# araffin/srl-zoo

Measured on AMD Instinct MI355X. Metric: images/sec (224x224x3) AE+VAE train step, higher is better.
Workload: dtype f32; 1 GPU; synthetic 224x224x3 obs, --losses autoencoder, custom_cnn, state-dim 200, bs=256 per GPU (512 frames fwd+bwd per step per GPU), Adam lr 0.005, normalised fp32 observations resident in HBM; global_batch=256, parallelism=dp1, rccl_ranks=1, devices=1

## Files before the change

include/srlz.h:

```cpp
#ifndef SRLZ_H
#define SRLZ_H

#include <stddef.h>
#include <stdint.h>

#ifdef __cplusplus
extern "C" {
#endif

typedef void* srlz_stream_t;

enum srlz_status {
  SRLZ_OK = 0,
  SRLZ_ERR_BAD_DESC = -1,
  SRLZ_ERR_WORKSPACE = -2,
  SRLZ_ERR_HIP = -3,
  SRLZ_ERR_NULL = -4
};

#define SRLZ_ABI_VERSION 104
int srlz_version(void);
const char* srlz_last_error(void);
int srlz_device_cus(void);

typedef struct {
  int n;
  int hi, wi;
  int ho, wo;
  int ksize;
  int stride;
  int pad;
  int transposed;
  int groups;
} srlz_conv64_desc;

size_t srlz_conv64_packed_floats(void);
int srlz_conv64_pack_weights(const float* w_ref, float* wpack_fwd, float* wpack_bwd,
                             const srlz_conv64_desc* d, srlz_stream_t stream);
int srlz_conv64_fwd_tiles(const srlz_conv64_desc* d);
int srlz_conv64_fwd(const float* x, const float* wpack_fwd, const float* bias, float* y, float* stats_partial,
                    const float* x_bnp, const srlz_conv64_desc* d, srlz_stream_t stream);
typedef struct {
  const float* y;
  const float* bnp;
  const float* sums;
  long long count;
  int training;
  float* dy_out;
} srlz_bn_bwd_operand;
int srlz_conv64_bwd_data(const float* dy, const float* wpack_bwd, float* dx, const srlz_bn_bwd_operand* dy_bn,
                         const srlz_conv64_desc* d, srlz_stream_t stream);
struct srlz_pool_desc_s;
int srlz_conv64_bwd_data_tiles(const srlz_conv64_desc* d);
// ... 309 lines not shown
```

srl-zoo_amd/csrc/common.h:

```cpp
#pragma once
#include <hip/hip_runtime.h>
#include <stdint.h>
#include <stddef.h>
#include "../../include/srlz.h"

typedef float f32x4 __attribute__((ext_vector_type(4)));
typedef float f32x16 __attribute__((ext_vector_type(16)));

void srlz_set_error(const char* fmt, ...);
int srlz_hip_fail(hipError_t e, const char* what);

#define SRLZ_HIP(expr)                                   \
  do {                                                   \
    hipError_t _e = (expr);                              \
    if (_e != hipSuccess) return srlz_hip_fail(_e, #expr); \
  } while (0)

#define SRLZ_MAX_LDS(fn, bytes)                                                                                         \
  do {                                                                                                                  \
    static int srlz_lds_set_ = -1;                                                                                      \
    if ((int)(bytes) > srlz_lds_set_) {                                                                                 \
      SRLZ_HIP(hipFuncSetAttribute((const void*)(fn), hipFuncAttributeMaxDynamicSharedMemorySize, (int)(bytes)));      \
      srlz_lds_set_ = (int)(bytes);                                                                                     \
    }                                                                                                                   \
// ... 117 lines not shown
  __syncthreads();
  if (threadIdx.x < 128) {
    double s = 0.0;
#pragma unroll
    for (int r = 0; r < 16; ++r) s += sm[r][threadIdx.x];
    row[threadIdx.x] = (T)s;
  }
}

template <class F4, class F1>
__device__ __forceinline__ void for_each_quad(long long n, F4 quad, F1 one) {
  const long long n4 = n >> 2, stride = (long long)gridDim.x * blockDim.x, first = (long long)blockIdx.x * blockDim.x + threadIdx.x;
  for (long long i = first; i < n4; i += stride) quad(i);
  for (long long i = n4 * 4 + first; i < n; i += stride) one(i);
}
```

srl-zoo_amd/csrc/conv64.hip:

```cpp
#include "conv64_tile.h"
#include <stdlib.h>

static int floordiv(int a, int b) { return (a >= 0) ? a / b : -((-a + b - 1) / b); }

int conv64::build_program(Prog* P, int gather, int stride, int pad, int N, int Hs, int Ws, int Hd, int Wd, int G) {
  if (stride != 1 && stride != 2) return -1;
  if (G < 1 || N % G != 0) return -1;
  N /= G;
  P->N = N; P->Hs = Hs; P->Ws = Ws; P->Hd = Hd; P->Wd = Wd;
  P->G = G;
  P->src_gstride = (long long)N * Hs * Ws * 64;
  P->dst_gstride = (long long)N * Hd * Wd * 64;
  int kcls[3], kd[3];
  if (gather) {
    P->ss = stride; P->ds = 1;
    for (int k = 0; k < 3; ++k) {
      int t = k - pad;
      int c = ((t % stride) + stride) % stride;
      kcls[k] = c; kd[k] = (t - c) / stride;
    }
  } else {
    P->ss = 1; P->ds = stride;
    for (int k = 0; k < 3; ++k) {
      int py = (((k - pad) % stride) + stride) % stride;
// ... 361 lines not shown
}

template <int PSUM>
__global__ __launch_bounds__(256, 2) void conv64_dgrad_poolsum_kernel(const float* __restrict__ src,
                                                                     const float* __restrict__ wpack,
                                                                     float* __restrict__ dst,
                                                                     float* __restrict__ bn_bwd_partial, const ConvProg P,
                                                                     int ntiles, const PoolSum ps) {
  conv64_fwd_body<4, false, PSUM>(src, wpack, nullptr, dst, bn_bwd_partial, P, ntiles, SRLZ_NO_FUSE, ps);
}

__global__ void conv64_pack_kernel(const float* __restrict__ w_ref, float* __restrict__ pf, float* __restrict__ pb,
                                   int transposed) {
  const int id = blockIdx.x * blockDim.x + threadIdx.x;
  if (id >= NTAPS * 4096) return;
  const int tap = id >> 12, n = (id >> 6) & 63, k = id & 63;
  const int o = (tap * 64 + n) * 64 + ((((k >> 2) ^ (n & 15)) << 2) | (k & 3));
  const int fwd_idx = transposed ? ((k * 64 + n) * 9 + tap) : ((n * 64 + k) * 9 + tap);
  const int bwd_idx = transposed ? ((n * 64 + k) * 9 + tap) : ((k * 64 + n) * 9 + tap);
  if (pf) pf[o] = w_ref[fwd_idx];
  if (pb) pb[o] = w_ref[bwd_idx];
}

static int check_desc(const srlz_conv64_desc* d) {
  SRLZ_REQUIRE(d != nullptr, SRLZ_ERR_NULL, "conv64: null descriptor");
  SRLZ_REQUIRE(d->ksize == 3 && (d->stride == 1 || d->stride == 2) && d->n > 0, SRLZ_ERR_BAD_DESC,
               "conv64: only 3x3 stride 1/2 supported (k=%d s=%d)", d->ksize, d->stride);
  SRLZ_REQUIRE(d->groups >= 0 && (d->groups <= 1 || d->n % d->groups == 0), SRLZ_ERR_BAD_DESC,
               "conv64: n = %d is not a multiple of groups = %d", d->n, d->groups);
  int eho, ewo;
  if (!d->transposed) {
    eho = (d->hi + 2 * d->pad - 3) / d->stride + 1;
    ewo = (d->wi + 2 * d->pad - 3) / d->stride + 1;
  } else {
    eho = (d->hi - 1) * d->stride - 2 * d->pad + 3;
    ewo = (d->wi - 1) * d->stride - 2 * d->pad + 3;
// ... 55 lines not shown
  SRLZ_REQUIRE(rc == 0, SRLZ_ERR_BAD_DESC, "conv64: cannot build a grid program for this descriptor");
  return 0;
}

extern "C" size_t srlz_conv64_packed_floats(void) { return (size_t)NTAPS * 4096; }

extern "C" int srlz_conv64_pack_weights(const float* w_ref, float* wpack_fwd, float* wpack_bwd,
                                        const srlz_conv64_desc* d, srlz_stream_t stream) {
  if (int rc = check_desc(d)) return rc;
  SRLZ_REQUIRE(w_ref, SRLZ_ERR_NULL, "conv64_pack: null weights");
  SRLZ_LAUNCH(conv64_pack_kernel, dim3((NTAPS * 4096 + 255) / 256), dim3(256), 0, as_stream(stream), w_ref, wpack_fwd, wpack_bwd,
              d->transposed);
  return 0;
}

extern "C" int srlz_conv64_fwd_tiles(const srlz_conv64_desc* d) {
  ConvProg P;
  if (conv64::with_program(d, 0, &P)) return -1;
  return P.G * P.tpg;
}

extern "C" int srlz_conv64_fwd(const float* x, const float* wpack_fwd, const float* bias, float* y,
                               float* stats_partial, const float* x_bnp, const srlz_conv64_desc* d,
                               srlz_stream_t stream) {
  ConvProg P;
  if (int rc = conv64::with_program(d, 0, &P)) return rc;
  SRLZ_REQUIRE(x && wpack_fwd && y, SRLZ_ERR_NULL, "conv64_fwd: null pointer");
  return launch_fwd(x, wpack_fwd, bias, y, stats_partial, P, as_stream(stream), OpFuse{x_bnp, nullptr, nullptr, 0.f, 0, nullptr});
}

// ... 44 lines not shown
```

srl-zoo_amd/csrc/linear.hip:

```cpp
#include "common.h"

namespace {

constexpr int BR = 32;
constexpr int LD = 68;

__global__ __launch_bounds__(256) void gemm_strided_kernel(const float* __restrict__ A, long long sai, long long sar,
                                                          const float* __restrict__ B, long long sbr, long long sbj,
                                                          const float* __restrict__ bias, float* __restrict__ C, int I,
                                                          int J, int R, int relu, int rchunk, const float* __restrict__ res,
                                                          long long ldr) {
  __shared__ float As[2][BR][LD];
  __shared__ float Bs[2][BR][LD];
  const int tid = threadIdx.x, lane = tid & 63, wave = tid >> 6;
  const int h = lane >> 5, l31 = lane & 31;
  const int wi = wave & 1, wj = wave >> 1;
  const int i0 = blockIdx.y * 64, j0 = blockIdx.x * 64;
  f32x16 acc;
#pragma unroll
  for (int r = 0; r < 16; ++r) acc[r] = 0.f;

  const int rbeg = blockIdx.z * rchunk;
  const int rend = (rbeg + rchunk < R) ? rbeg + rchunk : R;
  C += (size_t)blockIdx.z * I * J;
// ... 52 lines not shown
#pragma unroll
  for (int r = 0; r < 16; ++r) {
    const int i = i0 + wi * 32 + (r & 3) + 8 * (r >> 2) + 4 * h;
    if (i < I && j < J) {
      float v = acc[r] + bj;
      if (relu) v = v > 0.f ? v : 0.f;
      if (res) v = __fadd_rn(v, res[(long long)i * ldr + j]);
      C[(long long)i * J + j] = v;
    }
  }
}

constexpr int TR = 64;
__device__ __forceinline__ int tile_key(int row) { return ((row & 3) << 2) | ((row >> 2) & 3); }

template <bool AI, bool BI>
__global__ __launch_bounds__(256, 2) void gemm_vec_kernel(const float* __restrict__ A, long long lda, const float* __restrict__ B,
                                                         long long ldb, const float* __restrict__ bias, float* __restrict__ C,
                                                         int I, int J, int R, int relu, int rchunk, const float* __restrict__ res,
                                                         long long ldr) {
  __shared__ __attribute__((aligned(16))) float As[2][64 * TR];
  __shared__ __attribute__((aligned(16))) float Bs[2][64 * TR];
  const int tid = threadIdx.x, lane = tid & 63, wave = tid >> 6;
  const int h = lane >> 5, l31 = lane & 31;
  const int wi = wave & 1, wj = wave >> 1;
  const int i0 = blockIdx.y * 64, j0 = blockIdx.x * 64;
  f32x16 acc;
#pragma unroll
  for (int r = 0; r < 16; ++r) acc[r] = 0.f;
  const int rbeg = blockIdx.z * rchunk;
  const int rend = (rbeg + rchunk < R) ? rbeg + rchunk : R;
  C += (size_t)blockIdx.z * I * J;

  f32x4 va[4], vb[4];
  unsigned ina = 0, inb = 0;
// ... 6 lines not shown
      long long off;
      bool ok;
      if (!along_row) {
        const int row = e >> 4, r = 4 * (e & 15);
        ok = row0 + row < nrow && r0 + r < rend;
        off = (long long)(row0 + row) * ld + (r0 + r);
      } else {
        const int r = 4 * (e >> 6) + (e & 3), row = 4 * ((e >> 2) & 15);
        ok = row0 + row < nrow && r0 + r < rend;
        off = (long long)(r0 + r) * ld + (row0 + row);
      }
      v[u] = *(const f32x4*)(P + (ok ? off : 0LL));
      in |= (ok ? 1u : 0u) << u;
    }
  };
  auto stash_one = [&](float* __restrict__ T, bool along_row, const f32x4 (&v)[4], unsigned in) {
#pragma unroll
    for (int u = 0; u < 4; ++u) {
      const int e = tid + 256 * u;
      const f32x4 x = ((in >> u) & 1u) ? v[u] : f32x4{0.f, 0.f, 0.f, 0.f};
      if (!along_row) {
        const int row = e >> 4, slot = e & 15;
        *(f32x4*)(T + row * TR + ((slot ^ tile_key(row)) << 2)) = x;
      } else {
        const int r = 4 * (e >> 6) + (e & 3), row = 4 * ((e >> 2) & 15);
#pragma unroll
        for (int c = 0; c < 4; ++c) T[(row + c) * TR + ((((r >> 2) ^ tile_key(row + c)) << 2) | (r & 3))] = x[c];
      }
    }
  };
  fetch_one(A, lda, AI, i0, I, rbeg, va, ina);
  fetch_one(B, ldb, BI, j0, J, rbeg, vb, inb);
  stash_one(As[0], AI, va, ina);
  stash_one(Bs[0], BI, vb, inb);
  __syncthreads();
  int buf = 0;
  const int arow = wi * 32 + l31, brow = wj * 32 + l31;
  const int akey = tile_key(arow), bkey = tile_key(brow);
  for (int r0 = rbeg; r0 < rend; r0 += TR) {
    const int rn = (r0 + TR < rend) ? r0 + TR : rend;
    fetch_one(A, lda, AI, i0, I, rn, va, ina);
    fetch_one(B, ldb, BI, j0, J, rn, vb, inb);
    __builtin_amdgcn_sched_barrier(0);
    const float* Ab = As[buf] + arow * TR;
    const float* Bb = Bs[buf] + brow * TR;
#pragma unroll
    for (int c = 0; c < TR / 8; ++c) {
      const f32x4 a = *(const f32x4*)(Ab + (((2 * c + h) ^ akey) << 2));
      const f32x4 b = *(const f32x4*)(Bb + (((2 * c + h) ^ bkey) << 2));
#pragma unroll
      for (int m = 0; m < 4; ++m) acc = __builtin_amdgcn_mfma_f32_32x32x2f32(a[m], b[m], acc, 0, 0, 0);
    }
    stash_one(As[buf ^ 1], AI, va, ina);
    stash_one(Bs[buf ^ 1], BI, vb, inb);
    __syncthreads();
    buf ^= 1;
  }
  const int j = j0 + wj * 32 + l31;
  float bj = bias ? bias[j < J ? j : 0] : 0.f;
  asm volatile("" : "+v"(bj));
#pragma unroll
  for (int r = 0; r < 16; ++r) {
    const int i = i0 + wi * 32 + (r & 3) + 8 * (r >> 2) + 4 * h;
    if (i < I && j < J) {
      float v = acc[r] + bj;
      if (relu) v = v > 0.f ? v : 0.f;
      if (res) v = __fadd_rn(v, res[(long long)i * ldr + j]);
      C[(long long)i * J + j] = v;
    }
  }
}

__global__ void splitk_combine_kernel(const float* __restrict__ partial, int nsplit, const float* __restrict__ bias,
                                      float* __restrict__ C, int I, int J, int relu, const float* __restrict__ res, long long ldr) {
  const int e = blockIdx.x * blockDim.x + threadIdx.x;
  if (e >= I * J) return;
  float s = 0.f;
  for (int z = 0; z < nsplit; ++z) s += partial[(size_t)z * I * J + e];
  if (bias) s += bias[e % J];
  if (relu) s = s > 0.f ? s : 0.f;
  if (res) s = __fadd_rn(s, res[(long long)(e / J) * ldr + e % J]);
  C[e] = s;
}

// ... 30 lines not shown
  if (s > R / 128) s = R / 128;
  if (s > 16) s = 16;
  while (s > 1 && (size_t)s * I * J * sizeof(float) > ws_bytes) --s;
  return s < 1 ? 1 : s;
}

static bool vec_ok(const float* P, long long s_row, long long s_r, int nrow, int R, bool* along_row, long long* ld) {
  if (((uintptr_t)P & 15) != 0 || R % 4 != 0) return false;
  if (s_r == 1 && s_row % 4 == 0) { *along_row = false; *ld = s_row; return true; }
  if (s_row == 1 && s_r % 4 == 0 && nrow % 4 == 0) { *along_row = true; *ld = s_r; return true; }
  return false;
}

static int launch(const float* A, long long sai, long long sar, const float* B, long long sbr, long long sbj,
                  const float* bias, float* C, int I, int J, int R, int relu, void* ws, size_t ws_bytes, hipStream_t st,
                  const float* res = nullptr, long long ldr = 0) {
  SRLZ_REQUIRE(I > 0 && J > 0 && R > 0, SRLZ_ERR_BAD_DESC, "linear: empty GEMM %dx%dx%d", I, J, R);
  bool ai = false, bi = false;
  long long lda = 0, ldb = 0;
  const bool vec = vec_ok(A, sai, sar, I, R, &ai, &lda) && vec_ok(B, sbj, sbr, J, R, &bi, &ldb);
  const int step = vec ? TR : BR;
  int splits = ws ? choose_splits(I, J, R, ws_bytes, vec) : 1;
  int rchunk = R, nz = 1;
  if (splits > 1) {
    rchunk = (R + splits - 1) / splits;
    rchunk = (rchunk + step - 1) / step * step;
    nz = (R + rchunk - 1) / rchunk;
  }
  const dim3 grid((J + 63) / 64, (I + 63) / 64, nz);
  const float* kbias = nz > 1 ? nullptr : bias;
  float* kC = nz > 1 ? (float*)ws : C;
  const int krelu = nz > 1 ? 0 : relu;
  const float* kres = nz > 1 ? nullptr : res;
  if (vec) {
#define SRLZ_VEC_LAUNCH(AIV, BIV) \
    SRLZ_LAUNCH((gemm_vec_kernel<AIV, BIV>), grid, dim3(256), 0, st, A, lda, B, ldb, kbias, kC, I, J, R, krelu, rchunk, kres, ldr)
    if (ai && bi) SRLZ_VEC_LAUNCH(true, true);
    else if (ai) SRLZ_VEC_LAUNCH(true, false);
    else if (bi) SRLZ_VEC_LAUNCH(false, true);
    else SRLZ_VEC_LAUNCH(false, false);
#undef SRLZ_VEC_LAUNCH
  } else {
    SRLZ_LAUNCH(gemm_strided_kernel, grid, dim3(256), 0, st, A, sai, sar, B, sbr, sbj, kbias, kC, I, J, R, krelu, rchunk, kres, ldr);
  }
  if (nz > 1) {
    SRLZ_LAUNCH(splitk_combine_kernel, dim3((I * J + 255) / 256), dim3(256), 0, st, (const float*)ws, nz, bias, C, I, J, relu, res, ldr);
  }
  return 0;
}

}

// ... 20 lines not shown
                                        void* ws, size_t ws_bytes, srlz_stream_t stream) {
  SRLZ_REQUIRE(dy && w && dx && res, SRLZ_ERR_NULL, "linear_bwd_data_res: null pointer");
  SRLZ_REQUIRE(Kout >= 1 && Kout <= K, SRLZ_ERR_BAD_DESC, "linear_bwd_data_res: %d of %d input columns", Kout, K);
  return launch(dy, N, 1, w, K, 1, nullptr, dx, M, Kout, N, 0, ws, ws_bytes, as_stream(stream), res, Kout);
}

extern "C" int srlz_linear_bwd_data(const float* dy, const float* w, float* dx, int M, int N, int K, void* ws,
                                    size_t ws_bytes, srlz_stream_t stream) {
  SRLZ_REQUIRE(dy && w && dx, SRLZ_ERR_NULL, "linear_bwd_data: null pointer");
  return launch(dy, N, 1, w, K, 1, nullptr, dx, M, K, N, 0, ws, ws_bytes, as_stream(stream));
}

extern "C" int srlz_linear_bwd_weight(const float* dy, const float* x, float* dw, float* db, int M, int N, int K,
                                      void* ws, size_t ws_bytes, srlz_stream_t stream) {
  SRLZ_REQUIRE(dy && x && dw, SRLZ_ERR_NULL, "linear_bwd_weight: null pointer");
  if (int rc = launch(dy, 1, N, x, K, 1, nullptr, dw, N, K, M, 0, ws, ws_bytes, as_stream(stream))) return rc;
  if (db) {
    SRLZ_LAUNCH(colsum_kernel, dim3((N + 63) / 64), dim3(256), 0, as_stream(stream), dy, db, M, N);
  }
  return 0;
}

extern "C" int srlz_relu_bwd_inplace(const float* y, float* dy, long long n, srlz_stream_t stream) {
  SRLZ_REQUIRE(y && dy, SRLZ_ERR_NULL, "relu_bwd: null pointer");
  long long blocks = (n + 255) / 256;
  if (blocks > 4096) blocks = 4096;
  if (blocks < 1) blocks = 1;
  SRLZ_LAUNCH(relu_bwd_kernel, dim3((int)blocks), dim3(256), 0, as_stream(stream), y, dy, n);
  return 0;
}
```

srl-zoo_amd/csrc/wino.hip:

```cpp
#include "common.h"

namespace {

typedef float f32x2 __attribute__((ext_vector_type(2)));
typedef unsigned u32x2 __attribute__((ext_vector_type(2)));

constexpr int WN_THREADS = 256;
constexpr int WN_TP = 32;
constexpr int WN_CHUNK = 16 * 4 * 64 * 4;
constexpr int WN_VCHUNK = 16 * 4 * WN_TP * 4;
constexpr int WN_VCOMP = 4 * WN_TP * 4;
constexpr unsigned WN_DROP = 0x80000000u;

struct WinoProg {
  int N, G;
  int H, W;
  int PA, PB;
  int ppi, ppg, tpg;
  unsigned mPPI, mPB;
  int sPPI, sPB;
  long long gstride;
};

__global__ void conv64_wino_pack_kernel(const float* __restrict__ w_ref, float* __restrict__ uf, float* __restrict__ ub) {
  const int id = blockIdx.x * blockDim.x + threadIdx.x;
  if (id >= 64 * 64) return;
  const int e = id & 3, m = (id >> 2) & 63, gq = (id >> 8) & 3, p = id >> 10;
  const int k = 16 * p + 4 * gq + e;
#pragma unroll
  for (int dir = 0; dir < 2; ++dir) {
    float* out = dir ? ub : uf;
    if (!out) continue;
    float gk[3][3];
#pragma unroll
    for (int ky = 0; ky < 3; ++ky)
#pragma unroll
      for (int kx = 0; kx < 3; ++kx)
        gk[ky][kx] = dir ? w_ref[((k * 64 + m) * 3 + (2 - ky)) * 3 + (2 - kx)] : w_ref[((m * 64 + k) * 3 + ky) * 3 + kx];
    float t[3][4];
#pragma unroll
    for (int ky = 0; ky < 3; ++ky) {
      t[ky][0] = gk[ky][0];
      t[ky][1] = 0.5f * (gk[ky][0] + gk[ky][1] + gk[ky][2]);
      t[ky][2] = 0.5f * (gk[ky][0] - gk[ky][1] + gk[ky][2]);
      t[ky][3] = gk[ky][2];
    }
#pragma unroll
    for (int nu = 0; nu < 4; ++nu) {
      const float u0 = t[0][nu];
      const float u1 = 0.5f * (t[0][nu] + t[1][nu] + t[2][nu]);
      const float u2 = 0.5f * (t[0][nu] - t[1][nu] + t[2][nu]);
      const float u3 = t[2][nu];
      const float u[4] = {u0, u1, u2, u3};
#pragma unroll
      for (int xi = 0; xi < 4; ++xi) out[(size_t)p * WN_CHUNK + (((xi * 4 + nu) * 4 + gq) * 64 + m) * 4 + e] = u[xi];
    }
  }
}

struct WinoRaw { f32x2 d[16]; f32x2 sc, sh; };

struct WinoPatch {
  unsigned vtop, vmid, vbot;
  bool lef, rig;
};

__device__ __forceinline__ void wn_patch(WinoPatch& wp, const WinoProg& P, int tile_in_group, int t_pt, int t_cp, int* ptab_slot) {
  const int pl = tile_in_group * WN_TP + t_pt;
  const bool ok = pl < P.ppg;
  const int n = fastdiv(pl, P.mPPI, P.sPPI);
  const int rem = pl - n * P.ppi;
  const int a = fastdiv(rem, P.mPB, P.sPB);
// ... 698 lines not shown
```

srl-zoo_amd/models/models.py:

```python
from __future__ import print_function, division, absolute_import

import torch as th
import torch.nn as nn

try:
    from preprocessing.preprocess import getNChannels
except ImportError:
    from ..preprocessing.preprocess import getNChannels

from srlz import hotpath, ops


def conv3x3(in_planes, out_planes, stride=1):
    return nn.Conv2d(in_planes, out_planes, kernel_size=3, stride=stride, padding=1, bias=False)


def _encoder_stack():
    spec = [(nn.Conv2d(getNChannels(), 64, kernel_size=7, stride=2, padding=3, bias=False), 1),
            (conv3x3(64, 64, stride=1), 0),
            (conv3x3(64, 64, stride=2), 0)]
    layers = []
    for conv, pool_pad in spec:
        layers += [conv, nn.BatchNorm2d(64), nn.ReLU(inplace=True), nn.MaxPool2d(kernel_size=3, stride=2, padding=pool_pad)]
    return nn.Sequential(*layers)
# ... 26 lines not shown
    if isinstance(out, tuple):
        halves = [ops.pair_split(t) for t in out]
        return tuple(h[0] for h in halves), tuple(h[1] for h in halves)
    return ops.pair_split(out)


class BaseModelAutoEncoder(BaseModelSRL):

    def __init__(self):
        super(BaseModelAutoEncoder, self).__init__()
        self.encoder_conv = _encoder_stack()
        self.decoder_conv = _decoder_stack()

    def _encodeConv(self, x, stat_sink=None):
        hotpath.require_gpu(x, "encoder")
        e = hotpath.encoder_forward(self.encoder_conv, x, self.training, stat_sink)
        return e.view(e.size(0), -1)

    def _decodeConv(self, z):
        return hotpath.decoder_forward(self.decoder_conv, z.view(z.size(0), 64, 6, 6), self.training)

    def getStates(self, observations):
        return self.encode(observations)

    def encode(self, x):
        raise NotImplementedError

    def decode(self, x):
        raise NotImplementedError

    def forward(self, x):
# ... 85 lines not shown
```

srl-zoo_amd/srlz/_cabi.py:

```python
import ctypes
import os
from ctypes import c_int, c_longlong, c_float, c_double, c_void_p, c_size_t, c_char_p, POINTER, Structure

_HERE = os.path.dirname(os.path.abspath(__file__))
LIB_PATH = os.path.join(_HERE, "libsrlz_hip.so")


ABI_VERSION = 104


class SrlzError(RuntimeError):
    pass


class Conv64Desc(Structure):
    _fields_ = [("n", c_int), ("hi", c_int), ("wi", c_int), ("ho", c_int), ("wo", c_int), ("ksize", c_int),
                ("stride", c_int), ("pad", c_int), ("transposed", c_int), ("groups", c_int)]


class SkinnyDesc(Structure):
    _fields_ = [("n", c_int), ("c", c_int), ("himg", c_int), ("wimg", c_int), ("hf", c_int), ("wf", c_int),
                ("kind", c_int), ("groups", c_int)]


class PoolDesc(Structure):
    _fields_ = [("n", c_int), ("h", c_int), ("w", c_int), ("hp", c_int), ("wp", c_int), ("pool_pad", c_int),
                ("out_nchw", c_int), ("groups", c_int)]


class ConvNDesc(Structure):
    _fields_ = [("n", c_int), ("hi", c_int), ("wi", c_int), ("ho", c_int), ("wo", c_int), ("cin", c_int), ("cout", c_int),
                ("ksize", c_int), ("stride", c_int), ("pad", c_int), ("groups", c_int)]

    def __init__(self, n, hi, wi, ho, wo, cin, cout, ksize, stride, pad, groups=1):
        super(ConvNDesc, self).__init__(n, hi, wi, ho, wo, cin, cout, ksize, stride, pad, groups)


class BnReplayItem(Structure):
    _fields_ = [("batch_stat", c_void_p), ("running_mean", c_void_p), ("running_var", c_void_p), ("num_batches_tracked", c_void_p)]


class BnBwdOperand(Structure):
    _fields_ = [("y", c_void_p), ("bnp", c_void_p), ("sums", c_void_p), ("count", c_longlong), ("training", c_int),
                ("dy_out", c_void_p)]


P = c_void_p
_BO = POINTER(BnBwdOperand)
_C64 = POINTER(Conv64Desc)
_SK = POINTER(SkinnyDesc)
_PD = POINTER(PoolDesc)
_CN = POINTER(ConvNDesc)

_PROTOS = {
    "srlz_version": (c_int, []),
    "srlz_last_error": (c_char_p, []),
    "srlz_device_cus": (c_int, []),
    "srlz_conv64_packed_floats": (c_size_t, []),
    "srlz_conv64_pack_weights": (c_int, [P, P, P, _C64, P]),
    "srlz_conv64_fwd_tiles": (c_int, [_C64]),
    "srlz_conv64_fwd": (c_int, [P, P, P, P, P, P, _C64, P]),
    "srlz_conv64_bwd_data": (c_int, [P, P, P, _BO, _C64, P]),
    "srlz_conv64_bwd_weight_workspace": (c_size_t, [_C64]),
    "srlz_conv64_bwd_fused_supported": (c_int, [_C64]),
    "srlz_conv64_gather_pipe_supported": (c_int, [_C64, c_int]),
    "srlz_conv64_bwd_fused_workspace": (c_size_t, [_C64]),
    "srlz_conv64_bwd_fused": (c_int, [P, P, P, _BO, P, P, P, P, P, P, c_size_t, _C64, P]),
    "srlz_conv64_bwd_fused_bn_rows": (c_int, [_C64]),
    "srlz_conv64_wino_supported": (c_int, [_C64]),
    "srlz_conv64_wino_packed_floats": (c_size_t, []),
    "srlz_conv64_wino_pack_weights": (c_int, [P, P, P, P]),
    "srlz_conv64_wino_tiles": (c_int, [_C64]),
    "srlz_conv64_wino_fwd": (c_int, [P, P, P, P, P, P, _C64, P]),
    "srlz_conv64_wino_bwd_data": (c_int, [P, P, P, _C64, P]),
# ... 204 lines not shown
```

srl-zoo_amd/srlz/hotpath.py:

```python
import os
import torch

from . import ops

TAPS = None


OBSERVE = None


def _observe(prefix, idx, t):
    if OBSERVE is not None:
        OBSERVE["%s.%d" % (prefix, idx)] = (t.detach(), tuple(t.grad_fn.saved_tensors) if t.grad_fn is not None else ())
    return t


def _tap(prefix, idx, t):
    if TAPS is not None and t.requires_grad:
        t.retain_grad()
        TAPS["%s.%d" % (prefix, idx)] = t
    return t


_FUSE_ENC_IN = True
# ... 8 lines not shown
_RECON = None


class recon_loss_into(object):
    def __init__(self, target, mean):
        self.target, self.mean, self.loss = target, bool(mean), None

    def __enter__(self):
        global _RECON
        self.prev, _RECON = _RECON, (self if _FUSE_RECON else None)
        return self

    def __exit__(self, *exc):
        global _RECON
        _RECON = self.prev
        return False


def _bn_args(bn):
    bn.running_mean._srlz_tick = bn.num_batches_tracked
    return bn.weight, bn.bias, bn.running_mean, bn.running_var


def encoder_forward(seq, x, training, stat_sink=None, name="encoder_conv"):
    conv1, bn1, conv2, bn2, conv3, bn3 = seq[0], seq[1], seq[4], seq[5], seq[8], seq[9]
    if not _FUSE_ENC_IN:
        x = ops.frames_as_float(x)
    link1 = ops.PoolLink() if TAPS is None else None
    link2 = ops.PoolLink() if TAPS is None else None
    if _FUSE_ENC_IN and not x.requires_grad:
        p, y = ops.EncInFn.apply(x, conv1.weight, *_bn_args(bn1), training, 1, stat_sink, link1)
        _tap(name, 0, y)
        _tap(name, 3, p)
        _observe(name, 3, p)
    else:
        y, st = ops.Conv1Fn.apply(x, conv1.weight, training)
        _tap(name, 0, y)
        p = _tap(name, 3, ops.BNReLUPoolFn.apply(y, st, *_bn_args(bn1), training, 1, False, stat_sink, link1))
        _observe(name, 3, p)
    y, st = ops.Conv64Fn.apply(p, conv2.weight, None, 1, 1, False, training, link1)
    _tap(name, 4, y)
    p = _observe(name, 7, _tap(name, 7, ops.BNReLUPoolFn.apply(y, st, *_bn_args(bn2), training, 0, False, stat_sink, link2)))
    y, st = ops.Conv64Fn.apply(p, conv3.weight, None, 2, 1, False, training, link2)
    _tap(name, 8, y)
    return _observe(name, 11, _tap(name, 11, ops.BNReLUPoolFn.apply(y, st, *_bn_args(bn3), training, 0, True, stat_sink)))


def replay_encoder_bn(seq, stats, group=0):
    bns = (seq[1], seq[5], seq[9])
    items = [(st[128 * group:128 * (group + 1)], bn.running_mean, bn.running_var, bn.num_batches_tracked) for bn, st in zip(bns, stats)]
    ops._ordered_bn_update([bn.running_mean for bn in bns], lambda: ops.bn_replay_many(items))


def decoder_forward(seq, z, training):
    a = ops.ToNHWCFn.apply(z)
    y, st = ops.Conv64Fn.apply(a, seq[0].weight, seq[0].bias, 2, 0, True, training)
    _tap("decoder_conv", 0, y)
    defer = _DEFER_BN_BWD and TAPS is None
    in_link = None
    for bi, ci in ((1, 3), (4, 6), (7, 9)):
        bn, conv = seq[bi], seq[ci]
        if TAPS is not None:
            _record_activation(bi + 1, y, st, bn, training)
        out_link = ops.BwdLink() if defer else None
        y, st = ops.DecBlockFn.apply(y, st, *_bn_args(bn), training, conv.weight, conv.bias, training, in_link, out_link)
        in_link = out_link
        _tap("decoder_conv", ci, y)
        _observe("decoder_conv", ci, y)
    bn, last = seq[10], seq[12]
    if TAPS is not None:
        _record_activation(11, y, st, bn, training)
# ... 165 lines not shown
```

srl-zoo_amd/srlz/ops.py:

```python
import weakref

import torch
from torch.autograd import Function

from . import _cabi as C
from ._cabi import ptr, stream, Conv64Desc, SkinnyDesc, PoolDesc, ConvNDesc

BN_EPS = 1e-5
BN_MOMENTUM = 0.1

_GROUPS = 1


class batch_groups(object):
    def __init__(self, groups):
        self.groups = int(groups)

    def __enter__(self):
        global _GROUPS
        self.prev, _GROUPS = _GROUPS, self.groups
        return self

    def __exit__(self, *exc):
        global _GROUPS
# ... 202 lines not shown

class PoolLink:

    def __init__(self):
        self.record = None
        self.partials = None

    def take_partials(self):
        p, self.partials, self.record = self.partials, None, None
        return p


_POOL_LINK = True


class Conv64Fn(Function):
    @staticmethod
    def forward(ctx, x, w, bias, stride, pad, transposed, want_stats, in_link=None):
        x, w = _check(x, "conv64 input"), _check(w, "conv64 weight")
        n, hi, wi, ch = x.shape
        assert ch == 64 and tuple(w.shape) == (64, 64, 3, 3)
        d = conv64_desc(n, hi, wi, stride, pad, transposed, cur_groups(want_stats))
        y = torch.empty((n, d.ho, d.wo, 64), dtype=torch.float32, device=x.device)
        ctx.wino = bool(C.conv64_wino_supported(d))
        if ctx.wino:
            packs = torch.empty((2, C.conv64_wino_packed_floats()), dtype=torch.float32, device=x.device)
            C.conv64_wino_pack_weights(ptr(w), ptr(packs[0]), ptr(packs[1]), stream())
            stats = torch.empty((C.conv64_wino_tiles(d), 128), dtype=torch.float32, device=x.device) if want_stats else None
            _launch("conv64_wino_kernel", _conv64_key(d, "fwd"), _conv64_flop(d),
                    lambda: C.conv64_wino_fwd(ptr(x), ptr(packs[0]), ptr(bias), ptr(y), ptr(stats), None, d, stream()))
        else:
            packs = torch.empty((2, C.conv64_packed_floats()), dtype=torch.float32, device=x.device)
            C.conv64_pack_weights(ptr(w), ptr(packs[0]), ptr(packs[1]), d, stream())
            stats = torch.empty((C.conv64_fwd_tiles(d), 128), dtype=torch.float32, device=x.device) if want_stats else None
            name = "conv64_gather_pipe_kernel" if (bias is None and C.conv64_gather_pipe_supported(d, 0)) else "conv64_fwd_kernel"
            _launch(name, _conv64_key(d, "fwd"), _conv64_flop(d),
                    lambda: C.conv64_fwd(ptr(x), ptr(packs[0]), ptr(bias), ptr(y), ptr(stats), None, d, stream()))
        ctx.save_for_backward(x, packs)
        ctx.desc = d
        ctx.has_bias = bias is not None
        ctx.needs_dx = ctx.needs_input_grad[0]
        ctx.params = (w, bias)
        ctx.in_link = in_link
        if stats is None:
            stats = torch.empty(0, device=x.device)
        ctx.mark_non_differentiable(stats)
        ctx.set_materialize_grads(False)
        return y, stats
# ... 31 lines not shown
                            lambda: C.conv64_wino_bwd_data_pool_sums(ptr(dy), ptr(packs[1]), ptr(dx), ptr(pooled), ptr(pbnp), ptr(py),
                                                                     ptr(pargmax), pd, ptr(part), d, stream()))
                else:
                    part = torch.empty((C.conv64_bwd_data_tiles(d), 128), dtype=torch.float32, device=x.device)
                    _launch("conv64_dgrad_poolsum_kernel", _conv64_key(d, "dgrad"), _conv64_flop(d),
                            lambda: C.conv64_bwd_data_pool_sums(ptr(dy), ptr(packs[1]), ptr(dx), ptr(pooled), ptr(pbnp), ptr(py),
                                                                ptr(pargmax), pd, ptr(part), d, stream()))
                link.partials = part
            elif ctx.wino:
                _launch("conv64_wino_kernel", _conv64_key(d, "dgrad"), _conv64_flop(d),
                        lambda: C.conv64_wino_bwd_data(ptr(dy), ptr(packs[1]), ptr(dx), d, stream()))
            else:
                _launch("conv64_gather_pipe_kernel" if C.conv64_gather_pipe_supported(d, 1) else "conv64_fwd_kernel",
                        _conv64_key(d, "dgrad"), _conv64_flop(d),
                        lambda: C.conv64_bwd_data(ptr(dy), ptr(packs[1]), ptr(dx), None, d, stream()))
        return dx, _give(ctx.params[0], dw), _give(ctx.params[1], db), None, None, None, None, None


_bn_last_update = {}


def _ordered_bn_update(running_mean, fn):
    rms = running_mean if isinstance(running_mean, (list, tuple)) else [running_mean]
    cur = torch.cuda.current_stream(rms[0].device)
    for rm in rms:
        prev = _bn_last_update.get(rm.data_ptr())
        if prev is not None and prev[0] != cur.cuda_stream:
            cur.wait_event(prev[1])
    fn()
    ev = torch.cuda.Event()
    ev.record(cur)
# ... 212 lines not shown
                        dy_out.data_ptr() if materialise else None)
    return op, dy_out, rec




class DecBlockFn(Function):

    @staticmethod
    def forward(ctx, y_prev, stats_prev, gamma, beta, running_mean, running_var, training, w, bias, want_stats,
                in_link=None, out_link=None):
        y_prev, w = _check(y_prev, "decoder block input"), _check(w, "convT weight")
        n, hi, wi, _ = y_prev.shape
        bnp, _ = _bn_params(stats_prev, n * hi * wi, gamma, beta, running_mean, running_var, training, y_prev.device)
        d = conv64_desc(n, hi, wi, 2, 0, True, cur_groups(training))
        packs = torch.empty((2, C.conv64_packed_floats()), dtype=torch.float32, device=y_prev.device)
        C.conv64_pack_weights(ptr(w), ptr(packs[0]), ptr(packs[1]), d, stream())
        y = torch.empty((n, d.ho, d.wo, 64), dtype=torch.float32, device=y_prev.device)
        stats = torch.empty((C.conv64_fwd_tiles(d), 128), dtype=torch.float32, device=y_prev.device) if want_stats else None
        _launch("conv64_fwd_kernel", _conv64_key(d, "fwd"), _conv64_flop(d),
                lambda: C.conv64_fwd(ptr(y_prev), ptr(packs[0]), ptr(bias), ptr(y), ptr(stats), ptr(bnp), d, stream()))
        ctx.save_for_backward(y_prev, bnp, packs)
        ctx.desc, ctx.training = d, training
        ctx.in_link, ctx.out_link = in_link, out_link
        ctx.params = (gamma, beta, w, bias)
        if stats is None:
            stats = torch.empty(0, device=y_prev.device)
        ctx.mark_non_differentiable(stats)
        ctx.set_materialize_grads(False)
        return y, stats

    @staticmethod
# ... 1088 lines not shown
```

Before: 44640 images/s.

## Batch conv weight packing into one launch and fold bias colsum into GEMM

```diff
diff --git a/include/srlz.h b/include/srlz.h
--- a/include/srlz.h
+++ b/include/srlz.h
@@ -37,6 +37,15 @@
 size_t srlz_conv64_packed_floats(void);
 int srlz_conv64_pack_weights(const float* w_ref, float* wpack_fwd, float* wpack_bwd,
                              const srlz_conv64_desc* d, srlz_stream_t stream);
+#define SRLZ_CONV64_PACK_MAX 8
+enum { SRLZ_PACK_CONV = 0, SRLZ_PACK_CONVT = 1, SRLZ_PACK_WINO = 2 };
+typedef struct {
+  const float* w_ref;
+  float* pack_fwd;
+  float* pack_bwd;
+  int kind;
+} srlz_conv64_pack_item;
+int srlz_conv64_pack_many(const srlz_conv64_pack_item* items, int n, srlz_stream_t stream);
 int srlz_conv64_fwd_tiles(const srlz_conv64_desc* d);
 int srlz_conv64_fwd(const float* x, const float* wpack_fwd, const float* bias, float* y, float* stats_partial,
                     const float* x_bnp, const srlz_conv64_desc* d, srlz_stream_t stream);
diff --git a/srl-zoo_amd/csrc/common.h b/srl-zoo_amd/csrc/common.h
--- a/srl-zoo_amd/csrc/common.h
+++ b/srl-zoo_amd/csrc/common.h
@@ -155,3 +155,50 @@
   for (long long i = first; i < n4; i += stride) quad(i);
   for (long long i = n4 * 4 + first; i < n; i += stride) one(i);
 }
+
+constexpr int PACK64_FLOATS = 9 * 4096;
+constexpr int WINO_CHUNK_FLOATS = 16 * 4 * 64 * 4;
+
+__device__ __forceinline__ void pack64_element(int id, const float* __restrict__ w_ref, float* __restrict__ pf, float* __restrict__ pb,
+                                               int transposed) {
+  const int tap = id >> 12, n = (id >> 6) & 63, k = id & 63;
+  const int o = (tap * 64 + n) * 64 + ((((k >> 2) ^ (n & 15)) << 2) | (k & 3));
+  const int fwd_idx = transposed ? ((k * 64 + n) * 9 + tap) : ((n * 64 + k) * 9 + tap);
+  const int bwd_idx = transposed ? ((n * 64 + k) * 9 + tap) : ((k * 64 + n) * 9 + tap);
+  if (pf) pf[o] = w_ref[fwd_idx];
+  if (pb) pb[o] = w_ref[bwd_idx];
+}
+
+__device__ __forceinline__ void wino_pack_element(int id, const float* __restrict__ w_ref, float* __restrict__ uf, float* __restrict__ ub) {
+  const int e = id & 3, m = (id >> 2) & 63, gq = (id >> 8) & 3, p = id >> 10;
+  const int k = 16 * p + 4 * gq + e;
+#pragma unroll
+  for (int dir = 0; dir < 2; ++dir) {
+    float* out = dir ? ub : uf;
+    if (!out) continue;
+    float gk[3][3];
+#pragma unroll
+    for (int ky = 0; ky < 3; ++ky)
+#pragma unroll
+      for (int kx = 0; kx < 3; ++kx)
+        gk[ky][kx] = dir ? w_ref[((k * 64 + m) * 3 + (2 - ky)) * 3 + (2 - kx)] : w_ref[((m * 64 + k) * 3 + ky) * 3 + kx];
+    float t[3][4];
+#pragma unroll
+    for (int ky = 0; ky < 3; ++ky) {
+      t[ky][0] = gk[ky][0];
+      t[ky][1] = 0.5f * (gk[ky][0] + gk[ky][1] + gk[ky][2]);
+      t[ky][2] = 0.5f * (gk[ky][0] - gk[ky][1] + gk[ky][2]);
+      t[ky][3] = gk[ky][2];
+    }
+#pragma unroll
+    for (int nu = 0; nu < 4; ++nu) {
+      const float u0 = t[0][nu];
+      const float u1 = 0.5f * (t[0][nu] + t[1][nu] + t[2][nu]);
+      const float u2 = 0.5f * (t[0][nu] - t[1][nu] + t[2][nu]);
+      const float u3 = t[2][nu];
+      const float u[4] = {u0, u1, u2, u3};
+#pragma unroll
+      for (int xi = 0; xi < 4; ++xi) out[(size_t)p * WINO_CHUNK_FLOATS + (((xi * 4 + nu) * 4 + gq) * 64 + m) * 4 + e] = u[xi];
+    }
+  }
+}
diff --git a/srl-zoo_amd/csrc/conv64.hip b/srl-zoo_amd/csrc/conv64.hip
--- a/srl-zoo_amd/csrc/conv64.hip
+++ b/srl-zoo_amd/csrc/conv64.hip
@@ -399,12 +399,21 @@
                                    int transposed) {
   const int id = blockIdx.x * blockDim.x + threadIdx.x;
   if (id >= NTAPS * 4096) return;
-  const int tap = id >> 12, n = (id >> 6) & 63, k = id & 63;
-  const int o = (tap * 64 + n) * 64 + ((((k >> 2) ^ (n & 15)) << 2) | (k & 3));
-  const int fwd_idx = transposed ? ((k * 64 + n) * 9 + tap) : ((n * 64 + k) * 9 + tap);
-  const int bwd_idx = transposed ? ((n * 64 + k) * 9 + tap) : ((k * 64 + n) * 9 + tap);
-  if (pf) pf[o] = w_ref[fwd_idx];
-  if (pb) pb[o] = w_ref[bwd_idx];
+  pack64_element(id, w_ref, pf, pb, transposed);
+}
+
+struct PackTable {
+  srlz_conv64_pack_item it[SRLZ_CONV64_PACK_MAX];
+  int first[SRLZ_CONV64_PACK_MAX + 1];
+  int n;
+};
+__global__ __launch_bounds__(256) void conv64_pack_many_kernel(const PackTable t) {
+  int i = 0;
+  while (i + 1 < t.n && (int)blockIdx.x >= t.first[i + 1]) ++i;
+  const srlz_conv64_pack_item it = t.it[i];
+  const int id = ((int)blockIdx.x - t.first[i]) * 256 + threadIdx.x;
+  if (it.kind == SRLZ_PACK_WINO) wino_pack_element(id, it.w_ref, it.pack_fwd, it.pack_bwd);
+  else pack64_element(id, it.w_ref, it.pack_fwd, it.pack_bwd, it.kind == SRLZ_PACK_CONVT);
 }
 
 static int check_desc(const srlz_conv64_desc* d) {
@@ -490,6 +499,26 @@
   return 0;
 }
 
+extern "C" int srlz_conv64_pack_many(const srlz_conv64_pack_item* items, int n, srlz_stream_t stream) {
+  SRLZ_REQUIRE(items && n >= 1 && n <= SRLZ_CONV64_PACK_MAX, SRLZ_ERR_BAD_DESC, "conv64_pack_many: %d items (1 .. %d)", n,
+               SRLZ_CONV64_PACK_MAX);
+  static_assert(PACK64_FLOATS == NTAPS * 4096 && PACK64_FLOATS % 256 == 0, "a direct pack is a whole number of blocks");
+  PackTable t;
+  t.n = n;
+  t.first[0] = 0;
+  for (int i = 0; i < n; ++i) {
+    const srlz_conv64_pack_item& it = items[i];
+    SRLZ_REQUIRE(it.w_ref && (it.pack_fwd || it.pack_bwd), SRLZ_ERR_NULL, "conv64_pack_many: item %d: null pointer", i);
+    SRLZ_REQUIRE(it.kind == SRLZ_PACK_CONV || it.kind == SRLZ_PACK_CONVT || it.kind == SRLZ_PACK_WINO, SRLZ_ERR_BAD_DESC,
+                 "conv64_pack_many: item %d: kind %d", i, it.kind);
+    t.it[i] = it;
+    t.first[i + 1] = t.first[i] + (it.kind == SRLZ_PACK_WINO ? 64 * 64 : PACK64_FLOATS) / 256;
+  }
+  for (int i = n; i < SRLZ_CONV64_PACK_MAX; ++i) { t.it[i] = items[0]; t.first[i + 1] = t.first[n]; }
+  SRLZ_LAUNCH(conv64_pack_many_kernel, dim3(t.first[n]), dim3(256), 0, as_stream(stream), t);
+  return 0;
+}
+
 extern "C" int srlz_conv64_fwd_tiles(const srlz_conv64_desc* d) {
   ConvProg P;
   if (conv64::with_program(d, 0, &P)) return -1;
diff --git a/srl-zoo_amd/csrc/linear.hip b/srl-zoo_amd/csrc/linear.hip
--- a/srl-zoo_amd/csrc/linear.hip
+++ b/srl-zoo_amd/csrc/linear.hip
@@ -90,11 +90,12 @@
 constexpr int TR = 64;
 __device__ __forceinline__ int tile_key(int row) { return ((row & 3) << 2) | ((row >> 2) & 3); }
 
-template <bool AI, bool BI>
+template <bool AI, bool BI, bool ROWSUM = false>
 __global__ __launch_bounds__(256, 2) void gemm_vec_kernel(const float* __restrict__ A, long long lda, const float* __restrict__ B,
                                                          long long ldb, const float* __restrict__ bias, float* __restrict__ C,
                                                          int I, int J, int R, int relu, int rchunk, const float* __restrict__ res,
-                                                         long long ldr) {
+                                                         long long ldr, float* __restrict__ rowsum) {
+  static_assert(!ROWSUM || BI, "the ones column is written by the transposing stash");
   __shared__ __attribute__((aligned(16))) float As[2][64 * TR];
   __shared__ __attribute__((aligned(16))) float Bs[2][64 * TR];
   const int tid = threadIdx.x, lane = tid & 63, wave = tid >> 6;
@@ -131,11 +132,12 @@
       in |= (ok ? 1u : 0u) << u;
     }
   };
-  auto stash_one = [&](float* __restrict__ T, bool along_row, const f32x4 (&v)[4], unsigned in) {
+  auto stash_one = [&](float* __restrict__ T, bool along_row, const f32x4 (&v)[4], unsigned in, int ones_row = -1) {
 #pragma unroll
     for (int u = 0; u < 4; ++u) {
       const int e = tid + 256 * u;
-      const f32x4 x = ((in >> u) & 1u) ? v[u] : f32x4{0.f, 0.f, 0.f, 0.f};
+      f32x4 x = ((in >> u) & 1u) ? v[u] : f32x4{0.f, 0.f, 0.f, 0.f};
+      if (along_row && 4 * ((e >> 2) & 15) == ones_row) x = f32x4{1.f, 0.f, 0.f, 0.f};
       if (!along_row) {
         const int row = e >> 4, slot = e & 15;
         *(f32x4*)(T + row * TR + ((slot ^ tile_key(row)) << 2)) = x;
@@ -148,8 +150,9 @@
   };
   fetch_one(A, lda, AI, i0, I, rbeg, va, ina);
   fetch_one(B, ldb, BI, j0, J, rbeg, vb, inb);
+  const int ones_row = ROWSUM ? J - j0 : -1;
   stash_one(As[0], AI, va, ina);
-  stash_one(Bs[0], BI, vb, inb);
+  stash_one(Bs[0], BI, vb, inb, ones_row);
   __syncthreads();
   int buf = 0;
   const int arow = wi * 32 + l31, brow = wj * 32 + l31;
@@ -169,7 +172,7 @@
       for (int m = 0; m < 4; ++m) acc = __builtin_amdgcn_mfma_f32_32x32x2f32(a[m], b[m], acc, 0, 0, 0);
     }
     stash_one(As[buf ^ 1], AI, va, ina);
-    stash_one(Bs[buf ^ 1], BI, vb, inb);
+    stash_one(Bs[buf ^ 1], BI, vb, inb, ones_row);
     __syncthreads();
     buf ^= 1;
   }
@@ -185,6 +188,7 @@
       if (res) v = __fadd_rn(v, res[(long long)i * ldr + j]);
       C[(long long)i * J + j] = v;
     }
+    if (ROWSUM && i < I && j == J) rowsum[i] = acc[r];
   }
 }
 
@@ -245,7 +249,7 @@
 
 static int launch(const float* A, long long sai, long long sar, const float* B, long long sbr, long long sbj,
                   const float* bias, float* C, int I, int J, int R, int relu, void* ws, size_t ws_bytes, hipStream_t st,
-                  const float* res = nullptr, long long ldr = 0) {
+                  const float* res = nullptr, long long ldr = 0, float* rowsum = nullptr, bool* rowsum_done = nullptr) {
   SRLZ_REQUIRE(I > 0 && J > 0 && R > 0, SRLZ_ERR_BAD_DESC, "linear: empty GEMM %dx%dx%d", I, J, R);
   bool ai = false, bi = false;
   long long lda = 0, ldb = 0;
@@ -258,15 +262,21 @@
     rchunk = (rchunk + step - 1) / step * step;
     nz = (R + rchunk - 1) / rchunk;
   }
-  const dim3 grid((J + 63) / 64, (I + 63) / 64, nz);
+  const bool with_rowsum = rowsum && vec && ai && bi && nz == 1;
+  if (rowsum_done) *rowsum_done = with_rowsum;
+  const dim3 grid((J + (with_rowsum ? 1 : 0) + 63) / 64, (I + 63) / 64, nz);
   const float* kbias = nz > 1 ? nullptr : bias;
   float* kC = nz > 1 ? (float*)ws : C;
   const int krelu = nz > 1 ? 0 : relu;
   const float* kres = nz > 1 ? nullptr : res;
   if (vec) {
 #define SRLZ_VEC_LAUNCH(AIV, BIV) \
-    SRLZ_LAUNCH((gemm_vec_kernel<AIV, BIV>), grid, dim3(256), 0, st, A, lda, B, ldb, kbias, kC, I, J, R, krelu, rchunk, kres, ldr)
-    if (ai && bi) SRLZ_VEC_LAUNCH(true, true);
+    SRLZ_LAUNCH((gemm_vec_kernel<AIV, BIV>), grid, dim3(256), 0, st, A, lda, B, ldb, kbias, kC, I, J, R, krelu, rchunk, kres, ldr, \
+                (float*)nullptr)
+    if (with_rowsum) {
+      SRLZ_LAUNCH((gemm_vec_kernel<true, true, true>), grid, dim3(256), 0, st, A, lda, B, ldb, kbias, kC, I, J, R, krelu, rchunk, kres,
+                  ldr, rowsum);
+    } else if (ai && bi) SRLZ_VEC_LAUNCH(true, true);
     else if (ai) SRLZ_VEC_LAUNCH(true, false);
     else if (bi) SRLZ_VEC_LAUNCH(false, true);
     else SRLZ_VEC_LAUNCH(false, false);
@@ -317,8 +327,9 @@
 extern "C" int srlz_linear_bwd_weight(const float* dy, const float* x, float* dw, float* db, int M, int N, int K,
                                       void* ws, size_t ws_bytes, srlz_stream_t stream) {
   SRLZ_REQUIRE(dy && x && dw, SRLZ_ERR_NULL, "linear_bwd_weight: null pointer");
-  if (int rc = launch(dy, 1, N, x, K, 1, nullptr, dw, N, K, M, 0, ws, ws_bytes, as_stream(stream))) return rc;
-  if (db) {
+  bool db_done = false;
+  if (int rc = launch(dy, 1, N, x, K, 1, nullptr, dw, N, K, M, 0, ws, ws_bytes, as_stream(stream), nullptr, 0, db, &db_done)) return rc;
+  if (db && !db_done) {
     SRLZ_LAUNCH(colsum_kernel, dim3((N + 63) / 64), dim3(256), 0, as_stream(stream), dy, db, M, N);
   }
   return 0;
diff --git a/srl-zoo_amd/csrc/wino.hip b/srl-zoo_amd/csrc/wino.hip
--- a/srl-zoo_amd/csrc/wino.hip
+++ b/srl-zoo_amd/csrc/wino.hip
@@ -7,7 +7,7 @@
 
 constexpr int WN_THREADS = 256;
 constexpr int WN_TP = 32;
-constexpr int WN_CHUNK = 16 * 4 * 64 * 4;
+constexpr int WN_CHUNK = WINO_CHUNK_FLOATS;
 constexpr int WN_VCHUNK = 16 * 4 * WN_TP * 4;
 constexpr int WN_VCOMP = 4 * WN_TP * 4;
 constexpr unsigned WN_DROP = 0x80000000u;
@@ -25,37 +25,7 @@
 __global__ void conv64_wino_pack_kernel(const float* __restrict__ w_ref, float* __restrict__ uf, float* __restrict__ ub) {
   const int id = blockIdx.x * blockDim.x + threadIdx.x;
   if (id >= 64 * 64) return;
-  const int e = id & 3, m = (id >> 2) & 63, gq = (id >> 8) & 3, p = id >> 10;
-  const int k = 16 * p + 4 * gq + e;
-#pragma unroll
-  for (int dir = 0; dir < 2; ++dir) {
-    float* out = dir ? ub : uf;
-    if (!out) continue;
-    float gk[3][3];
-#pragma unroll
-    for (int ky = 0; ky < 3; ++ky)
-#pragma unroll
-      for (int kx = 0; kx < 3; ++kx)
-        gk[ky][kx] = dir ? w_ref[((k * 64 + m) * 3 + (2 - ky)) * 3 + (2 - kx)] : w_ref[((m * 64 + k) * 3 + ky) * 3 + kx];
-    float t[3][4];
-#pragma unroll
-    for (int ky = 0; ky < 3; ++ky) {
-      t[ky][0] = gk[ky][0];
-      t[ky][1] = 0.5f * (gk[ky][0] + gk[ky][1] + gk[ky][2]);
-      t[ky][2] = 0.5f * (gk[ky][0] - gk[ky][1] + gk[ky][2]);
-      t[ky][3] = gk[ky][2];
-    }
-#pragma unroll
-    for (int nu = 0; nu < 4; ++nu) {
-      const float u0 = t[0][nu];
-      const float u1 = 0.5f * (t[0][nu] + t[1][nu] + t[2][nu]);
-      const float u2 = 0.5f * (t[0][nu] - t[1][nu] + t[2][nu]);
-      const float u3 = t[2][nu];
-      const float u[4] = {u0, u1, u2, u3};
-#pragma unroll
-      for (int xi = 0; xi < 4; ++xi) out[(size_t)p * WN_CHUNK + (((xi * 4 + nu) * 4 + gq) * 64 + m) * 4 + e] = u[xi];
-    }
-  }
+  wino_pack_element(id, w_ref, uf, ub);
 }
 
 struct WinoRaw { f32x2 d[16]; f32x2 sc, sh; };
diff --git a/srl-zoo_amd/models/models.py b/srl-zoo_amd/models/models.py
--- a/srl-zoo_amd/models/models.py
+++ b/srl-zoo_amd/models/models.py
@@ -64,7 +64,7 @@
 
     def _encodeConv(self, x, stat_sink=None):
         hotpath.require_gpu(x, "encoder")
-        e = hotpath.encoder_forward(self.encoder_conv, x, self.training, stat_sink)
+        e = hotpath.encoder_forward(self.encoder_conv, x, self.training, stat_sink, decoder=self.decoder_conv)
         return e.view(e.size(0), -1)
 
     def _decodeConv(self, z):
diff --git a/srl-zoo_amd/srlz/_cabi.py b/srl-zoo_amd/srlz/_cabi.py
--- a/srl-zoo_amd/srlz/_cabi.py
+++ b/srl-zoo_amd/srlz/_cabi.py
@@ -38,6 +38,14 @@
 
 class BnReplayItem(Structure):
     _fields_ = [("batch_stat", c_void_p), ("running_mean", c_void_p), ("running_var", c_void_p), ("num_batches_tracked", c_void_p)]
+
+
+class Conv64PackItem(Structure):
+    _fields_ = [("w_ref", c_void_p), ("pack_fwd", c_void_p), ("pack_bwd", c_void_p), ("kind", c_int)]
+
+
+PACK_CONV, PACK_CONVT, PACK_WINO = 0, 1, 2
+CONV64_PACK_MAX = 8
 
 
 class BnBwdOperand(Structure):
@@ -58,6 +66,7 @@
     "srlz_device_cus": (c_int, []),
     "srlz_conv64_packed_floats": (c_size_t, []),
     "srlz_conv64_pack_weights": (c_int, [P, P, P, _C64, P]),
+    "srlz_conv64_pack_many": (c_int, [POINTER(Conv64PackItem), c_int, P]),
     "srlz_conv64_fwd_tiles": (c_int, [_C64]),
     "srlz_conv64_fwd": (c_int, [P, P, P, P, P, P, _C64, P]),
     "srlz_conv64_bwd_data": (c_int, [P, P, P, _BO, _C64, P]),
diff --git a/srl-zoo_amd/srlz/hotpath.py b/srl-zoo_amd/srlz/hotpath.py
--- a/srl-zoo_amd/srlz/hotpath.py
+++ b/srl-zoo_amd/srlz/hotpath.py
@@ -46,6 +46,7 @@
     def __exit__(self, *exc):
         global _RECON
         _RECON = self.prev
+        ops.drop_prepacked()
         return False
 
 
@@ -54,8 +55,16 @@
     return bn.weight, bn.bias, bn.running_mean, bn.running_var
 
 
-def encoder_forward(seq, x, training, stat_sink=None, name="encoder_conv"):
+def _decoder_packs(seq):
+    return [(seq[ci].weight, ops.C.PACK_CONVT) for ci in (0, 3, 6, 9)]
+
+
+def encoder_forward(seq, x, training, stat_sink=None, name="encoder_conv", decoder=None):
     conv1, bn1, conv2, bn2, conv3, bn3 = seq[0], seq[1], seq[4], seq[5], seq[8], seq[9]
+    ops.drop_prepacked()
+    pack_with = [(conv3.weight, ops.C.PACK_CONV)]
+    if decoder is not None and _RECON is not None:
+        pack_with += _decoder_packs(decoder)
     if not _FUSE_ENC_IN:
         x = ops.frames_as_float(x)
     link1 = ops.PoolLink() if TAPS is None else None
@@ -70,7 +79,7 @@
         _tap(name, 0, y)
         p = _tap(name, 3, ops.BNReLUPoolFn.apply(y, st, *_bn_args(bn1), training, 1, False, stat_sink, link1))
         _observe(name, 3, p)
-    y, st = ops.Conv64Fn.apply(p, conv2.weight, None, 1, 1, False, training, link1)
+    y, st = ops.Conv64Fn.apply(p, conv2.weight, None, 1, 1, False, training, link1, pack_with)
     _tap(name, 4, y)
     p = _observe(name, 7, _tap(name, 7, ops.BNReLUPoolFn.apply(y, st, *_bn_args(bn2), training, 0, False, stat_sink, link2)))
     y, st = ops.Conv64Fn.apply(p, conv3.weight, None, 2, 1, False, training, link2)
@@ -86,7 +95,7 @@
 
 def decoder_forward(seq, z, training):
     a = ops.ToNHWCFn.apply(z)
-    y, st = ops.Conv64Fn.apply(a, seq[0].weight, seq[0].bias, 2, 0, True, training)
+    y, st = ops.Conv64Fn.apply(a, seq[0].weight, seq[0].bias, 2, 0, True, training, None, _decoder_packs(seq)[1:])
     _tap("decoder_conv", 0, y)
     defer = _DEFER_BN_BWD and TAPS is None
     in_link = None
diff --git a/srl-zoo_amd/srlz/ops.py b/srl-zoo_amd/srlz/ops.py
--- a/srl-zoo_amd/srlz/ops.py
+++ b/srl-zoo_amd/srlz/ops.py
@@ -240,9 +240,40 @@
 _POOL_LINK = True
 
 
+_PREPACKED = {}
+
+
+def drop_prepacked():
+    _PREPACKED.clear()
+
+
+def _packs64(w, kind, d=None, pack_with=None):
+    hit = _PREPACKED.pop(w.data_ptr(), None)
+    if hit is not None and hit[0] == w._version and hit[1] == kind:
+        return hit[2]
+    others = [(ow, ok) for ow, ok in (pack_with or ()) if ow.data_ptr() != w.data_ptr() and ow.is_cuda and ow.device == w.device
+              and ow.dtype == torch.float32 and ow.is_contiguous() and tuple(ow.shape) == (64, 64, 3, 3)][:C.CONV64_PACK_MAX - 1]
+    floats = lambda k: C.conv64_wino_packed_floats() if k == C.PACK_WINO else C.conv64_packed_floats()
+    packs = torch.empty((2, floats(kind)), dtype=torch.float32, device=w.device)
+    if not others:
+        if kind == C.PACK_WINO:
+            C.conv64_wino_pack_weights(ptr(w), ptr(packs[0]), ptr(packs[1]), stream())
+        else:
+            C.conv64_pack_weights(ptr(w), ptr(packs[0]), ptr(packs[1]), d, stream())
+        return packs
+    todo = [(w, kind, packs)] + [(ow, ok, torch.empty((2, floats(ok)), dtype=torch.float32, device=w.device)) for ow, ok in others]
+    table = (C.Conv64PackItem * len(todo))()
+    for i, (ow, ok, pk) in enumerate(todo):
+        table[i].w_ref, table[i].pack_fwd, table[i].pack_bwd, table[i].kind = ow.data_ptr(), pk[0].data_ptr(), pk[1].data_ptr(), ok
+    C.conv64_pack_many(table, len(todo), stream())
+    for ow, ok, pk in todo[1:]:
+        _PREPACKED[ow.data_ptr()] = (ow._version, ok, pk)
+    return packs
+
+
 class Conv64Fn(Function):
     @staticmethod
-    def forward(ctx, x, w, bias, stride, pad, transposed, want_stats, in_link=None):
+    def forward(ctx, x, w, bias, stride, pad, transposed, want_stats, in_link=None, pack_with=None):
         x, w = _check(x, "conv64 input"), _check(w, "conv64 weight")
         n, hi, wi, ch = x.shape
         assert ch == 64 and tuple(w.shape) == (64, 64, 3, 3)
@@ -250,14 +281,12 @@
         y = torch.empty((n, d.ho, d.wo, 64), dtype=torch.float32, device=x.device)
         ctx.wino = bool(C.conv64_wino_supported(d))
         if ctx.wino:
-            packs = torch.empty((2, C.conv64_wino_packed_floats()), dtype=torch.float32, device=x.device)
-            C.conv64_wino_pack_weights(ptr(w), ptr(packs[0]), ptr(packs[1]), stream())
+            packs = _packs64(w, C.PACK_WINO, None, pack_with)
             stats = torch.empty((C.conv64_wino_tiles(d), 128), dtype=torch.float32, device=x.device) if want_stats else None
             _launch("conv64_wino_kernel", _conv64_key(d, "fwd"), _conv64_flop(d),
                     lambda: C.conv64_wino_fwd(ptr(x), ptr(packs[0]), ptr(bias), ptr(y), ptr(stats), None, d, stream()))
         else:
-            packs = torch.empty((2, C.conv64_packed_floats()), dtype=torch.float32, device=x.device)
-            C.conv64_pack_weights(ptr(w), ptr(packs[0]), ptr(packs[1]), d, stream())
+            packs = _packs64(w, C.PACK_CONVT if transposed else C.PACK_CONV, d, pack_with)
             stats = torch.empty((C.conv64_fwd_tiles(d), 128), dtype=torch.float32, device=x.device) if want_stats else None
             name = "conv64_gather_pipe_kernel" if (bias is None and C.conv64_gather_pipe_supported(d, 0)) else "conv64_fwd_kernel"
             _launch(name, _conv64_key(d, "fwd"), _conv64_flop(d),
@@ -319,7 +348,7 @@
                 _launch("conv64_gather_pipe_kernel" if C.conv64_gather_pipe_supported(d, 1) else "conv64_fwd_kernel",
                         _conv64_key(d, "dgrad"), _conv64_flop(d),
                         lambda: C.conv64_bwd_data(ptr(dy), ptr(packs[1]), ptr(dx), None, d, stream()))
-        return dx, _give(ctx.params[0], dw), _give(ctx.params[1], db), None, None, None, None, None
+        return dx, _give(ctx.params[0], dw), _give(ctx.params[1], db), None, None, None, None, None, None
 
 
 _bn_last_update = {}
@@ -562,8 +591,7 @@
         n, hi, wi, _ = y_prev.shape
         bnp, _ = _bn_params(stats_prev, n * hi * wi, gamma, beta, running_mean, running_var, training, y_prev.device)
         d = conv64_desc(n, hi, wi, 2, 0, True, cur_groups(training))
-        packs = torch.empty((2, C.conv64_packed_floats()), dtype=torch.float32, device=y_prev.device)
-        C.conv64_pack_weights(ptr(w), ptr(packs[0]), ptr(packs[1]), d, stream())
+        packs = _packs64(w, C.PACK_CONVT, d)
         y = torch.empty((n, d.ho, d.wo, 64), dtype=torch.float32, device=y_prev.device)
         stats = torch.empty((C.conv64_fwd_tiles(d), 128), dtype=torch.float32, device=y_prev.device) if want_stats else None
         _launch("conv64_fwd_kernel", _conv64_key(d, "fwd"), _conv64_flop(d),
```

After: 44810 images/s (median of 6 runs). No clear change (+0.4%).
